# ov2slam/ov2slam

Hardware: AMD Instinct MI355X
Metric: frames/sec tracking + local-BA iters/sec, EuRoC MH_01 stereo 'accurate', 1 GPU vs CPU ref (higher is better)
Workload: dtype u8/int32 fixed point + f32 (LK), f64 (BA)

## Files before the change

ov2slam_amd/csrc/clahe.hip:

```cpp
#include "common.hpp"
#include "xcd_map.hpp"
#include <math.h>
#include <mutex>
#include <type_traits>

#pragma clang fp contract(off)

__device__ __forceinline__ int c_reflect101(int p, int len)
{
    if (len == 1) return 0;
    while (p < 0 || p >= len) p = p < 0 ? -p : 2 * len - 2 - p;
    return p;
}

struct ClaheParams {
    int w, h, stride, tiles_x, tiles_y, tw, th, clip;
    float lut_scale, inv_tw, inv_th;
    long long src_item_stride, dst_item_stride;
    int dst_stride;
    int border;
    int batch, gx_lut;
    int ysplit;
    int nstrips, nlut;
    long long l1_delta;
    int l1_pitch, l1_w, l1_h;
};

__device__ __forceinline__ void clahe_wave_sync()
{
    __builtin_amdgcn_fence(__ATOMIC_RELEASE, "wavefront");
    __builtin_amdgcn_wave_barrier();
    __builtin_amdgcn_fence(__ATOMIC_ACQUIRE, "wavefront");
}

#define CH_WAVE_DW 256
#define CH_CSTRIDE 264
#define CH_NCOPY 4
#define CH_MULTI_DW (CH_NCOPY * CH_CSTRIDE)
typedef uint32_t c_u32x4 __attribute__((ext_vector_type(4)));

template <int CTRL>
__device__ __forceinline__ int c_dpp0(int v) { return __builtin_amdgcn_update_dpp(0, v, CTRL, 0xF, 0xF, true); }

template <bool SRC_ALIGNED, class StoreLut>
__device__ __forceinline__ void clahe_lut_tiles(const ClaheParams &P, const uint8_t *img, uint32_t *hw, int lane, int t, int t_end, int tstride,
                                                StoreLut store_lut, int ncopy = 1)
{
    const int ntiles = t_end;
    const int sub = lane >> 4, l16 = lane & 15;
    uint32_t *hist = hw + ((lane ^ (lane >> 4)) & (ncopy - 1)) * CH_CSTRIDE;
    const bool fast_geom = P.tw <= 61 && P.th <= 64;
    const uint8_t *img_end = img + (long long)(P.h - 1) * P.stride + P.w;
    const bool same_phase = SRC_ALIGNED || (P.stride & 3) == 0;

    auto tile_fast = [&](int t) { const int xb = (t % P.tiles_x) * P.tw; return fast_geom && 2 * xb + P.tw <= 2 * P.w - 1; };
    const uint32_t lane_off = (uint32_t)(sub * P.stride + 4 * l16);
    auto tile_load = [&](int t, uint32_t (&vv)[16], uint32_t &phs) {
        const int ty = t / P.tiles_x, tx = t - ty * P.tiles_x;
        const int x_begin = tx * P.tw;
        if (SRC_ALIGNED && (ty * P.th + 64 <= P.h) && (long long)P.h * P.stride < (1ll << 31)) {
            const uint32_t ph = (uint32_t)(x_begin & 3);
            phs = ph * 0x55555555u;
            const uint8_t *tp = img + (long long)(ty * P.th) * P.stride + (x_begin & ~3);
            uint32_t off = (4 * l16 < P.tw + (int)ph && (x_begin & ~3) + 4 * l16 < P.w) ? lane_off : (uint32_t)(sub * P.stride);
#pragma unroll
            for (int i = 0; i < 16; i++) {
                vv[i] = *(const uint32_t *)(tp + off);
                off += 4u * (uint32_t)P.stride;
            }
            return;
        }
        const int ybase = ty * P.th + sub;
        phs = 0;
#pragma unroll
        for (int i = 0; i < 16; i++) {
            int y = ybase + 4 * i;
            y = y >= P.h ? 2 * P.h - 2 - y : y;
            y = y < 0 ? 0 : y;
            uint32_t v = 0;
            if (SRC_ALIGNED) {
                const uint32_t ph = (uint32_t)(x_begin & 3);
                phs |= ph << (2 * i);
                if (4 * i + sub < P.th && 4 * l16 < P.tw + (int)ph && (x_begin & ~3) + 4 * l16 < P.w) v = *(const uint32_t *)(img + y * P.stride + (x_begin & ~3) + 4 * l16);
            } else {
                const uint8_t *rp = img + (long long)y * P.stride + x_begin;
                const uint32_t ph = (uint32_t)((size_t)rp & 3);
                phs |= ph << (2 * i);
                const uint8_t *ap = rp - ph + 4 * l16;
                if (4 * i + sub < P.th && 4 * l16 < P.tw + (int)ph && x_begin - (int)ph + 4 * l16 < P.w) {
                    if (ap + 4 <= img_end) v = *(const uint32_t *)ap;
                    else for (int k = 0; k < 4; k++) if (ap + k < img_end) v |= (uint32_t)ap[k] << (8 * k);
                }
            }
            vv[i] = v;
        }
    };

    uint32_t cur[16], cur_ph = 0;
    auto histogram = [&](int th) {
        const int ty = th / P.tiles_x, tx = th - ty * P.tiles_x;
        const int x_begin = tx * P.tw;
        if (ncopy == 1) ((c_u32x4 *)hw)[lane] = (c_u32x4)(0u);
        else for (int q = lane; q < CH_MULTI_DW / 4; q += 64) ((c_u32x4 *)hw)[q] = (c_u32x4)(0u);
        clahe_wave_sync();
        if (tile_fast(th)) {
            const int dbl_lo = 2 * P.w - 2 - (x_begin + P.tw);
            auto wgt = [&](int p) { const int c = x_begin + p; return ((unsigned)p < (unsigned)P.tw && c < P.w) ? ((c > dbl_lo && c <= P.w - 2) ? 2u : 1u) : 0u; };
            const int p_same = 4 * l16 - (int)(cur_ph & 3);
            uint32_t w0 = wgt(p_same), w1 = wgt(p_same + 1), w2 = wgt(p_same + 2), w3 = wgt(p_same + 3);
            bool mine = p_same < P.tw;
#pragma unroll
            for (int i = 0; i < 16; i++) {
                if (!same_phase) {
                    const int p0 = 4 * l16 - (int)((cur_ph >> (2 * i)) & 3);
                    w0 = wgt(p0); w1 = wgt(p0 + 1); w2 = wgt(p0 + 2); w3 = wgt(p0 + 3);
                    mine = p0 < P.tw;
                }
                if (mine && 4 * i + sub < P.th) {
                    const uint32_t v = cur[i];
                    atomicAdd(&hist[v & 0xFF], w0);
                    atomicAdd(&hist[(v >> 8) & 0xFF], w1);
                    atomicAdd(&hist[(v >> 16) & 0xFF], w2);
                    atomicAdd(&hist[v >> 24], w3);
                }
            }
        } else {
            for (int ly = sub; ly < P.th; ly += 4) {
                const uint8_t *row = img + (long long)c_reflect101(ty * P.th + ly, P.h) * P.stride;
                for (int lx = l16; lx < P.tw; lx += 16) atomicAdd(&hist[row[c_reflect101(x_begin + lx, P.w)]], 1u);
            }
        }
    };
    if (t < ntiles) {
        if (tile_fast(t)) tile_load(t, cur, cur_ph);
        histogram(t);
        if (t + tstride < ntiles && tile_fast(t + tstride)) tile_load(t + tstride, cur, cur_ph);
    }
#pragma nounroll
    for (; t < ntiles; t += tstride) {
        clahe_wave_sync();
        int hv[4];
        {
            c_u32x4 q = *(const c_u32x4 *)(hw + 4 * lane);
            for (int c = 1; c < ncopy; c++) q += *(const c_u32x4 *)(hw + c * CH_CSTRIDE + 4 * lane);
            hv[0] = (int)q.x; hv[1] = (int)q.y; hv[2] = (int)q.z; hv[3] = (int)q.w;
        }
        clahe_wave_sync();
        const int tn = t + tstride;
        if (tn < ntiles) {
            histogram(tn);
            if (tn + tstride < ntiles && tile_fast(tn + tstride)) tile_load(tn + tstride, cur, cur_ph);
        }
        if (P.clip > 0) {
            int over = 0;
#pragma unroll
            for (int k = 0; k < 4; k++) { over += max(hv[k] - P.clip, 0); hv[k] = min(hv[k], P.clip); }
            over += c_dpp0<0xB1>(over); over += c_dpp0<0x4E>(over); over += c_dpp0<0x124>(over); over += c_dpp0<0x128>(over);
            const int clipped = __builtin_amdgcn_readlane(over, 0) + __builtin_amdgcn_readlane(over, 16) +
                                __builtin_amdgcn_readlane(over, 32) + __builtin_amdgcn_readlane(over, 48);
            const int batch = clipped >> 8, residual = clipped & 255;
            int step = residual ? (int)(256.0f / (float)residual) : 1;
            int q = (int)((float)(4 * lane) / (float)step), r = 4 * lane - q * step;
#pragma unroll
            for (int k = 0; k < 4; k++) {
                hv[k] += batch + ((residual != 0 && r == 0 && q < residual) ? 1 : 0);
                r++;
                if (r == step) { r = 0; q++; }
            }
        }
        hv[1] += hv[0]; hv[2] += hv[1]; hv[3] += hv[2];
        int v = hv[3];
        v += c_dpp0<0x111>(v); v += c_dpp0<0x112>(v); v += c_dpp0<0x114>(v); v += c_dpp0<0x118>(v);
        const int r0 = __builtin_amdgcn_readlane(v, 15), r1 = __builtin_amdgcn_readlane(v, 31), r2 = __builtin_amdgcn_readlane(v, 47);
        const int rowoff = sub == 0 ? 0 : (sub == 1 ? r0 : (sub == 2 ? r0 + r1 : r0 + r1 + r2));
        const int base = v + rowoff - hv[3];
        uint32_t packed = 0;
#pragma unroll
        for (int k = 0; k < 4; k++) {
            int r = __float2int_rn((float)(hv[k] + base) * P.lut_scale);
            r = r < 0 ? 0 : (r > 255 ? 255 : r);
            packed |= (uint32_t)r << (8 * k);
        }
        store_lut(t, packed);
    }
}

template <bool SRC_ALIGNED>
__global__ __launch_bounds__(256, 4) void k_clahe_lut(ClaheParams P, const uint8_t *__restrict__ src, uint8_t *__restrict__ lut)
{
    __shared__ __attribute__((aligned(16))) uint32_t hist_all[4][CH_MULTI_DW];
    const int wave = __builtin_amdgcn_readfirstlane(threadIdx.x >> 6), lane = threadIdx.x & 63;
    const int ntiles = P.tiles_x * P.tiles_y;
    int b, bx;
    ov2_xcd_map(blockIdx.x, P.gx_lut, P.batch, &b, &bx);
    uint8_t *lb = lut + (long long)b * ntiles * 256 + 4 * lane;
    clahe_lut_tiles<SRC_ALIGNED>(P, src + (long long)b * P.src_item_stride, hist_all[wave], lane, bx * 4 + wave, ntiles, 4 * P.gx_lut,
                                 [&](int t, uint32_t packed) { *(uint32_t *)(lb + (long long)t * 256) = packed; }, CH_NCOPY);
}

#define CLAHE_MAX_CELLS 48
#define CA_UNROLL 6
typedef float c_f32x2 __attribute__((ext_vector_type(2)));

__device__ __forceinline__ float c_ub(uint32_t q, int k) { return (float)((q >> (8 * k)) & 0xFFu); }

template <bool SRC_ALIGNED>
__global__ __launch_bounds__(512) void k_clahe_apply(ClaheParams P, const uint8_t *__restrict__ src, const uint8_t *__restrict__ lut,
                                                     uint8_t *__restrict__ dst)
{
    extern __shared__ __align__(16) unsigned char clahe_smem[];
    const int ncx = P.tiles_x + 1;
    uint32_t *lut4 = (uint32_t *)clahe_smem;
    int cy, b;
    ov2_xcd_map(blockIdx.x, (P.tiles_y + 1) * P.ysplit, P.batch, &b, &cy);
    const int part = cy % P.ysplit;
    cy /= P.ysplit;
    const int tid = threadIdx.x, nthr = blockDim.x;
    const int ty1 = max(cy - 1, 0), ty2 = min(cy, P.tiles_y - 1);
    const uint8_t *L = lut + (long long)b * P.tiles_x * P.tiles_y * 256;
    for (int e = tid; e < ncx * 64; e += nthr) {
        const int cx = e >> 6, v4 = (e & 63) * 4;
        const int tx1 = max(cx - 1, 0), tx2 = min(cx, P.tiles_x - 1);
        const uint32_t a = *(const uint32_t *)(L + (ty1 * P.tiles_x + tx1) * 256 + v4), bb = *(const uint32_t *)(L + (ty1 * P.tiles_x + tx2) * 256 + v4);
        const uint32_t c = *(const uint32_t *)(L + (ty2 * P.tiles_x + tx1) * 256 + v4), d = *(const uint32_t *)(L + (ty2 * P.tiles_x + tx2) * 256 + v4);
        const uint32_t ab01 = __builtin_amdgcn_perm(bb, a, 0x05010400u), ab23 = __builtin_amdgcn_perm(bb, a, 0x07030602u);
        const uint32_t cd01 = __builtin_amdgcn_perm(d, c, 0x05010400u), cd23 = __builtin_amdgcn_perm(d, c, 0x07030602u);
        c_u32x4 o;
        o.x = __builtin_amdgcn_perm(cd01, ab01, 0x05040100u); o.y = __builtin_amdgcn_perm(cd01, ab01, 0x07060302u);
        o.z = __builtin_amdgcn_perm(cd23, ab23, 0x05040100u); o.w = __builtin_amdgcn_perm(cd23, ab23, 0x07060302u);
        *(c_u32x4 *)(lut4 + (cx << 8) + v4) = o;
    }
    __syncthreads();
    int y0 = max(0, (int)floorf(((float)cy - 0.5f) * (float)P.th) - 1), y1 = min(P.h, (int)ceilf(((float)cy + 0.5f) * (float)P.th) + 2);
    while (y0 < y1 && (int)floorf((float)y0 * P.inv_th - 0.5f) + 1 != cy) y0++;
    while (y1 > y0 && (int)floorf((float)(y1 - 1) * P.inv_th - 0.5f) + 1 != cy) y1--;
    if (P.ysplit > 1) {
        const int chunk = (y1 - y0 + P.ysplit - 1) / P.ysplit;
        y0 = min(y1, y0 + part * chunk);
        y1 = min(y1, y0 + chunk);
    }
    const uint8_t *simg = src + (long long)b * P.src_item_stride;
    uint8_t *dimg = dst + (long long)b * P.dst_item_stride;
    const bool dst_aligned = ((P.dst_stride | (int)(size_t)dimg) & 3) == 0;
    constexpr bool src_aligned = SRC_ALIGNED;
    const uint8_t *simg_end = simg + (long long)(P.h - 1) * P.stride + P.w;
    const int ndw = (P.w + 3) >> 2;
    for (int dwi = tid; dwi < ndw; dwi += nthr) {
        const int xb = 4 * dwi;
        float xa[4], xa1[4];
        const uint32_t *lutc[4];
#pragma unroll
        for (int k = 0; k < 4; k++) {
            const int x = min(xb + k, P.w - 1);
            const float txf = (float)x * P.inv_tw - 0.5f;
            const int fx = (int)floorf(txf);
            xa[k] = txf - (float)fx; xa1[k] = 1.0f - xa[k];
            lutc[k] = lut4 + ((fx + 1) << 8);
        }
        const c_f32x2 XA01 = {xa[0], xa[1]}, XA23 = {xa[2], xa[3]}, XB01 = {xa1[0], xa1[1]}, XB23 = {xa1[2], xa1[3]};
        const bool full = dst_aligned && xb + 3 < P.w;
        auto load_rows = [&](int yb, uint32_t (&inr)[CA_UNROLL]) {
#pragma unroll
            for (int u = 0; u < CA_UNROLL; u++) {
                const int y = min(yb + u, y1 - 1);
                const uint8_t *sp = simg + (long long)y * P.stride + xb;
                uint32_t in = 0;
                if (src_aligned) in = *(const uint32_t *)sp;
                else {
                    const uint32_t ph = (uint32_t)((size_t)sp & 3);
                    const uint8_t *ap = sp - ph;
                    if (xb + 3 < P.w && ap + 8 <= simg_end) {
                        const uint32_t lo = *(const uint32_t *)ap, hi = *(const uint32_t *)(ap + 4);
                        in = __builtin_amdgcn_alignbyte(hi, lo, ph);
                    } else for (int k = 0; k < 4; k++) if (xb + k < P.w) in |= (uint32_t)sp[k] << (8 * k);
                }
                inr[u] = in;
            }
        };
        uint32_t inr[CA_UNROLL], nxt[CA_UNROLL];
        if (y0 < y1) load_rows(y0, inr);
        for (int yb = y0; yb < y1; yb += CA_UNROLL) {
            load_rows(yb + CA_UNROLL, nxt);
#pragma unroll
            for (int u = 0; u < CA_UNROLL; u++) {
                const int y = yb + u;
                if (y >= y1) break;
                const float tyf = (float)y * P.inv_th - 0.5f;
                const float ya = tyf - (float)(cy - 1), ya1 = 1.0f - ya;
                const c_f32x2 YA = {ya, ya}, YB = {ya1, ya1};
                uint8_t *drow = dimg + y * P.dst_stride;
                const uint32_t in = inr[u];
                const uint32_t q0 = lutc[0][in & 0xFF], q1 = lutc[1][(in >> 8) & 0xFF], q2 = lutc[2][(in >> 16) & 0xFF], q3 = lutc[3][in >> 24];
                const c_f32x2 A11 = {c_ub(q0, 0), c_ub(q1, 0)}, A12 = {c_ub(q0, 1), c_ub(q1, 1)}, A21 = {c_ub(q0, 2), c_ub(q1, 2)}, A22 = {c_ub(q0, 3), c_ub(q1, 3)};
                const c_f32x2 B11 = {c_ub(q2, 0), c_ub(q3, 0)}, B12 = {c_ub(q2, 1), c_ub(q3, 1)}, B21 = {c_ub(q2, 2), c_ub(q3, 2)}, B22 = {c_ub(q2, 3), c_ub(q3, 3)};
                const c_f32x2 r01 = (A11 * XB01 + A12 * XA01) * YB + (A21 * XB01 + A22 * XA01) * YA;
                const c_f32x2 r23 = (B11 * XB23 + B12 * XA23) * YB + (B21 * XB23 + B22 * XA23) * YA;
                uint32_t out = __builtin_amdgcn_cvt_pk_u8_f32(rintf(r01.x), 0, 0u);
                out = __builtin_amdgcn_cvt_pk_u8_f32(rintf(r01.y), 1, out);
                out = __builtin_amdgcn_cvt_pk_u8_f32(rintf(r23.x), 2, out);
                out = __builtin_amdgcn_cvt_pk_u8_f32(rintf(r23.y), 3, out);
                if (full) *(uint32_t *)(drow + xb) = out;
                else for (int k = 0; k < 4; k++) if (xb + k < P.w) drow[xb + k] = (uint8_t)(out >> (8 * k));
            }
#pragma unroll
            for (int u = 0; u < CA_UNROLL; u++) inr[u] = nxt[u];
        }
    }
    if (P.border > 0) {
        __threadfence_block();
        __syncthreads();
        const int win = P.border, pbl = (win + 3) & ~3, wend = (P.w + win + 3) & ~3, rbeg = P.w & ~3;
        const int ndw_lr = pbl / 4 + ((wend - rbeg) >> 2), ndw_row = (pbl + wend) >> 2;
        auto put = [&](int yt, int ysrc, int c0) {
            const uint8_t *srow = dimg + ysrc * P.dst_stride;
            uint32_t v;
            if (c0 >= 0 && c0 + 3 < P.w) v = *(const uint32_t *)(srow + c0);
            else {
                v = 0;
#pragma unroll
                for (int k = 0; k < 4; k++) {
                    int c = c0 + k;
                    c = c < -win ? -win : (c > P.w + win - 1 ? P.w + win - 1 : c);
                    v |= (uint32_t)srow[c_reflect101(c, P.w)] << (8 * k);
                }
            }
            *(uint32_t *)(dimg + yt * P.dst_stride + c0) = v;
        };
        for (int row = tid >> 3; row < y1 - y0; row += nthr >> 3)
            for (int d = tid & 7; d < ndw_lr; d += 8)
                put(y0 + row, y0 + row, d < pbl / 4 ? 4 * d - pbl : rbeg + 4 * (d - pbl / 4));
        for (int k = max(1, y0); k <= min(win, y1 - 1); k++)
            for (int d = tid; d < ndw_row; d += nthr) put(-k, k, 4 * d - pbl);
        for (int k = max(1, P.h - y1); k <= min(win, P.h - 1 - y0); k++)
            for (int d = tid; d < ndw_row; d += nthr) put(P.h - 1 + k, P.h - 1 - k, 4 * d - pbl);
    }
}

__device__ __forceinline__ uint32_t c_wave_shr1(uint32_t v) { return (uint32_t)__builtin_amdgcn_update_dpp(0, (int)v, 0x138, 0xF, 0xF, true); }
__device__ __forceinline__ uint32_t c_wave_shl1(uint32_t v) { return (uint32_t)__builtin_amdgcn_update_dpp(0, (int)v, 0x130, 0xF, 0xF, true); }

#define CS_UNROLL 6
#define CS_MAX_STRIPS 8
#define CS_LUT_PRIO 3
template <bool UNAL, bool FUSED>
__global__ __launch_bounds__(64 * (CS_MAX_STRIPS + 2), 6) void k_clahe_apply_pyr(ClaheParams P, const uint8_t *__restrict__ src, const uint8_t *__restrict__ lut,
                                                                                uint8_t *__restrict__ dst)
{
    extern __shared__ __align__(16) unsigned char clahe_smem[];
    uint32_t *lut4 = (uint32_t *)clahe_smem;
    uint8_t *ring = clahe_smem + (size_t)(P.tiles_x + 1) * 1024;
    const int b = blockIdx.x, s = __builtin_amdgcn_readfirstlane(threadIdx.x >> 6);
    const int lane = threadIdx.x & 63, ndw = (P.w + 3) >> 2, wr = UNAL ? (P.w & 3) : 0;
    uint32_t *hist_w = (uint32_t *)(ring + (size_t)2 * P.tiles_x * 256) + (s < P.nstrips ? s * CH_WAVE_DW : P.nstrips * CH_WAVE_DW + (s - P.nstrips) * CH_MULTI_DW);
    const int hist_copies = s < P.nstrips ? 1 : CH_NCOPY;
    auto lut_row = [&](int ty, int tx0, int txstep) {
        uint8_t *slot = ring + (size_t)(ty & 1) * P.tiles_x * 256 - (size_t)ty * P.tiles_x * 256 + 4 * lane;
        clahe_lut_tiles<!UNAL>(P, src + (long long)b * P.src_item_stride, hist_w, lane, ty * P.tiles_x + tx0, (ty + 1) * P.tiles_x, txstep,
                               [&](int t, uint32_t packed) { *(uint32_t *)(slot + (size_t)t * 256) = packed; }, hist_copies);
    };
    typedef uint32_t cs_u32_a1 __attribute__((aligned(1)));
    const int cmin = 0, ncell = P.tiles_x + 1;
    const uint8_t *L = lut + (long long)b * P.tiles_x * P.tiles_y * 256;
    auto cell_row = [&](int y) { return (int)floorf((float)y * P.inv_th - 0.5f) + 1; };
    int cy = -1, y_switch = 0;
    auto build = [&](int cyv) {
        const int ty1 = max(cyv - 1, 0), ty2 = min(cyv, P.tiles_y - 1);
        const uint8_t *L1 = FUSED ? ring + (size_t)(ty1 & 1) * P.tiles_x * 256 : L + (size_t)ty1 * P.tiles_x * 256;
        const uint8_t *L2 = FUSED ? ring + (size_t)(ty2 & 1) * P.tiles_x * 256 : L + (size_t)ty2 * P.tiles_x * 256;
        __syncthreads();
        for (int e = threadIdx.x; e < ncell * 64; e += blockDim.x) {
            const int cx = cmin + (e >> 6), v4 = (e & 63) * 4;
            const int tx1 = max(cx - 1, 0), tx2 = min(cx, P.tiles_x - 1);
            const uint32_t a = *(const uint32_t *)(L1 + tx1 * 256 + v4), bb = *(const uint32_t *)(L1 + tx2 * 256 + v4);
            const uint32_t c = *(const uint32_t *)(L2 + tx1 * 256 + v4), dd = *(const uint32_t *)(L2 + tx2 * 256 + v4);
            const uint32_t ab01 = __builtin_amdgcn_perm(bb, a, 0x05010400u), ab23 = __builtin_amdgcn_perm(bb, a, 0x07030602u);
            const uint32_t cd01 = __builtin_amdgcn_perm(dd, c, 0x05010400u), cd23 = __builtin_amdgcn_perm(dd, c, 0x07030602u);
            c_u32x4 o;
            o.x = __builtin_amdgcn_perm(cd01, ab01, 0x05040100u); o.y = __builtin_amdgcn_perm(cd01, ab01, 0x07060302u);
            o.z = __builtin_amdgcn_perm(cd23, ab23, 0x05040100u); o.w = __builtin_amdgcn_perm(cd23, ab23, 0x07060302u);
            *(c_u32x4 *)(lut4 + ((e >> 6) << 8) + v4) = o;
        }
        __syncthreads();
    };
    if (FUSED) {
        lut_row(0, s, P.nstrips + P.nlut);
        if (s >= P.nstrips) {
            const int n_cell_rows = cell_row(P.h - 1) + 1;
            __builtin_amdgcn_s_setprio(CS_LUT_PRIO);
            for (int c = 0; c < n_cell_rows; c++) {
                build(c);
                if (c + 1 < P.tiles_y) lut_row(c + 1, s - P.nstrips, P.nlut);
            }
            return;
        }
    }
    const int core0 = s == 0 ? 0 : 63 + 62 * (s - 1);
    const int core1 = s == P.nstrips - 1 ? ndw : 63 + 62 * s;
    const int d_first = s == 0 ? 0 : core0 - 1;
    const int d_raw = d_first + lane;
    const int d = min(d_raw, ndw - 1);
    const bool core = d_raw >= core0 && d_raw < core1;
    const int xb = 4 * d;
    float xa[4], xa1[4];
    const uint32_t *lutc[4];
#pragma unroll
    for (int k = 0; k < 4; k++) {
        const float txf = (float)min(xb + k, P.w - 1) * P.inv_tw - 0.5f;
        const int fx = (int)floorf(txf);
        xa[k] = txf - (float)fx; xa1[k] = 1.0f - xa[k];
        lutc[k] = lut4 + ((fx + 1 - cmin) << 8);
    }
    const c_f32x2 XA01 = {xa[0], xa[1]}, XA23 = {xa[2], xa[3]}, XB01 = {xa1[0], xa1[1]}, XB23 = {xa1[2], xa1[3]};
    uint8_t *dimg = dst + (long long)b * P.dst_item_stride;
    uint8_t *l1 = dimg + P.l1_delta;
    const int win = P.border;
    const int l1odd = UNAL ? (P.l1_w & 1) : 0;
    const int nb0 = (win + 3) >> 2, nb1 = (win + 1) >> 1;
    const int nbr0 = nb0 + (wr ? 1 : 0), nbr1 = nb1 + l1odd;
    const bool bl0 = core && d < nb0, br0 = core && d >= ndw - nbr0;
    const bool bl1 = core && d >= 1 && d <= nb1, br1 = core && d >= ndw - nbr1;
    const bool edge_strip = s == 0 || core1 > ndw - max(nbr0, nbr1);
    const bool first_col = d_raw == 0, last_col = d_raw == ndw - 1;
    const bool dup = d_raw > ndw - 1;
    const uint32_t pad0 = 4u * nb0, pad1 = 2u * nb1;
    const uint32_t slack0 = pad0 + 4u * (uint32_t)((P.w + win + 3) >> 2), slack1 = pad1 + 2u * (uint32_t)((P.l1_w + win + 3) >> 1);
    const uint32_t o0 = dup ? slack0 : pad0 + 4u * d;
    const uint32_t o0b = bl0 ? pad0 - 4u * (d + 1) : (br0 ? pad0 + (uint32_t)(2 * P.w - 2 - xb - ((wr & 1) ? 0 : 2)) : slack0);
    const uint32_t sel_br = (wr & 1) ? 0x01020304u : 0x03040506u;
    const uint32_t sel_fix = (last_col && wr) ? (wr == 1 ? 0x01020304u : (wr == 2 ? 0x03040504u : 0x05060504u)) : 0x07060504u;
    const uint32_t sel_rt = wr == 0 ? 0x0c0c0c06u : (wr == 1 ? 0x0c0c0c00u : (wr == 2 ? 0x0c0c0c02u : 0x0c0c0c04u));
    const uint32_t o1 = core ? pad1 + 2u * d : slack1;
    const uint32_t o1b = bl1 ? pad1 - 2u * d : (br1 ? pad1 + (uint32_t)P.l1_w + 2u * (ndw - 1 - d) - (uint32_t)l1odd : slack1);
    const bool fix1 = last_col && l1odd;
    uint8_t *d0m = dimg - pad0, *d1m = l1 - pad1;
    const uint32_t xo = (d == ndw - 1 && wr) ? (uint32_t)(P.w - 4) : (uint32_t)xb;
    const uint32_t in_sh = (d == ndw - 1 && wr) ? 8u * (4u - (uint32_t)wr) : 0u;

    auto stage = [&](int y) {
        cy = cell_row(y);
        int yn = max(y + 1, (int)(((float)cy + 0.5f) * (float)P.th) - 2);
        while (yn < P.h && cell_row(yn) == cy) yn++;
        y_switch = yn;
        build(cy);
    };
    uint8_t *dbase = min(d0m - (long long)win * P.dst_stride, d1m - (long long)win * P.l1_pitch) - 256;
    const __amdgpu_buffer_rsrc_t rs_dst = __builtin_amdgcn_make_buffer_rsrc(dbase, 0, 0x7fffffff, 0x00020000);
    const uint8_t *sbase = src + (long long)b * P.src_item_stride;
    const __amdgpu_buffer_rsrc_t rs_src = __builtin_amdgcn_make_buffer_rsrc((void *)sbase, 0, 0x7fffffff, 0x00020000);
    auto put0 = [&](uint8_t *row, uint32_t v, uint32_t bv) {
        const int so = (int)(row - dbase);
        __builtin_amdgcn_raw_buffer_store_b32(v, rs_dst, (int)o0, so, 0);
        if (edge_strip) __builtin_amdgcn_raw_buffer_store_b32(bv, rs_dst, (int)o0b, so, 0);
    };
    auto put1 = [&](uint8_t *row, uint32_t v, uint32_t bv) {
        const int so = (int)(row - dbase);
        __builtin_amdgcn_raw_buffer_store_b16((unsigned short)v, rs_dst, (int)o1, so, 0);
        if (edge_strip) __builtin_amdgcn_raw_buffer_store_b16((unsigned short)bv, rs_dst, (int)o1b, so, 0);
    };
    typedef unsigned short cu16x2 __attribute__((ext_vector_type(2)));
    uint8_t *r1 = d1m;
    auto emit = [&](int Y, uint32_t c0, uint32_t c1, uint32_t c2, uint32_t c3, uint32_t c4, auto mirror_c) {
        constexpr bool MIRROR = decltype(mirror_c)::value;
        const cu16x2 s0 = __builtin_bit_cast(cu16x2, c0), s1 = __builtin_bit_cast(cu16x2, c1), s2 = __builtin_bit_cast(cu16x2, c2),
                     s3 = __builtin_bit_cast(cu16x2, c3), s4 = __builtin_bit_cast(cu16x2, c4);
        const cu16x2 v = (s2 * (unsigned short)6 + (s1 + s3) * (unsigned short)4 + s0 + s4 + (unsigned short)128) >> (unsigned short)8;
        uint32_t o = __builtin_amdgcn_perm(0u, __builtin_bit_cast(uint32_t, v), 0x0c0c0200u);
        uint32_t bv = 0;
        if (edge_strip) {
            bv = __builtin_amdgcn_perm(c_wave_shr1(o), o, 0x0c0c0500u);
            if (UNAL && fix1) o = bv;
        }
        put1(r1, o, bv);
        r1 += P.l1_pitch;
        if (MIRROR) {
            if (Y >= 1 && Y <= win) put1(d1m - (long long)Y * P.l1_pitch, o, bv);
            if (Y >= P.l1_h - 1 - win && Y <= P.l1_h - 2) put1(d1m + (long long)(2 * (P.l1_h - 1) - Y) * P.l1_pitch, o, bv);
        }
    };

    uint32_t hA = 0, hB = 0, hC = 0, hD = 0, hE = 0;
    const uint8_t *srow = src + (long long)b * P.src_item_stride;
    uint8_t *r0 = d0m;
    uint32_t inr[CS_UNROLL], nxt[CS_UNROLL];
#pragma unroll
    for (int u = 0; u < CS_UNROLL; u++) inr[u] = *(const cs_u32_a1 *)(srow + (long long)min(u, P.h - 1) * P.stride + xo) >> (UNAL ? in_sh : 0u);
    srow += (long long)CS_UNROLL * P.stride;
    auto do_row = [&](int y, uint32_t in, auto mirror_c) {
        constexpr bool MIRROR = decltype(mirror_c)::value;
        const float tyf = (float)y * P.inv_th - 0.5f;
        const float ya = tyf - (float)(cy - 1), ya1 = 1.0f - ya;
        const c_f32x2 YA = {ya, ya}, YB = {ya1, ya1};
        const uint32_t q0 = lutc[0][in & 0xFF], q1 = lutc[1][(in >> 8) & 0xFF], q2 = lutc[2][(in >> 16) & 0xFF], q3 = lutc[3][in >> 24];
        const c_f32x2 A11 = {c_ub(q0, 0), c_ub(q1, 0)}, A12 = {c_ub(q0, 1), c_ub(q1, 1)}, A21 = {c_ub(q0, 2), c_ub(q1, 2)}, A22 = {c_ub(q0, 3), c_ub(q1, 3)};
        const c_f32x2 B11 = {c_ub(q2, 0), c_ub(q3, 0)}, B12 = {c_ub(q2, 1), c_ub(q3, 1)}, B21 = {c_ub(q2, 2), c_ub(q3, 2)}, B22 = {c_ub(q2, 3), c_ub(q3, 3)};
        const c_f32x2 r01 = (A11 * XB01 + A12 * XA01) * YB + (A21 * XB01 + A22 * XA01) * YA;
        const c_f32x2 r23 = (B11 * XB23 + B12 * XA23) * YB + (B21 * XB23 + B22 * XA23) * YA;
        const c_f32x2 MAGIC = {12582912.0f, 12582912.0f};
        const c_f32x2 m01 = r01 + MAGIC, m23 = r23 + MAGIC;
        const uint32_t u0 = __builtin_bit_cast(uint32_t, (float)m01.x), u1 = __builtin_bit_cast(uint32_t, (float)m01.y);
        const uint32_t u2 = __builtin_bit_cast(uint32_t, (float)m23.x), u3 = __builtin_bit_cast(uint32_t, (float)m23.y);
        uint32_t out = __builtin_amdgcn_perm(__builtin_amdgcn_perm(u3, u2, 0x0c0c0400u), __builtin_amdgcn_perm(u1, u0, 0x0c0c0400u), 0x05040100u);
        uint32_t lf = c_wave_shr1(out), rt = c_wave_shl1(out);
        if (first_col) lf = __builtin_amdgcn_perm(out, out, 0x01020000u);
        if (edge_strip) {
            if (UNAL) out = __builtin_amdgcn_perm(out, lf, sel_fix);
        }
        if (UNAL) { if (last_col) rt = __builtin_amdgcn_perm(out, lf, sel_rt); }
        else if (last_col) rt = out >> 16;
        uint32_t bv = 0;
        if (edge_strip)
            bv = bl0 ? __builtin_amdgcn_perm(out, rt, 0x05060700u) : __builtin_amdgcn_perm(out, lf, sel_br);
        put0(r0, out, bv);
        r0 += P.dst_stride;
        if (MIRROR) {
            if (y >= 1 && y <= win) put0(d0m - (long long)y * P.dst_stride, out, bv);
            if (y >= P.h - 1 - win && y <= P.h - 2) put0(d0m + (long long)(2 * (P.h - 1) - y) * P.dst_stride, out, bv);
        }
        const uint32_t l0 = __builtin_amdgcn_alignbyte(out, lf, 2);
        const uint32_t h0 = __builtin_amdgcn_udot4(l0, 0x04060401u, __builtin_amdgcn_udot4(out, 0x00010000u, 0u, false), false);
        const uint32_t h1 = __builtin_amdgcn_udot4(out, 0x04060401u, __builtin_amdgcn_udot4(rt, 0x00000001u, 0u, false), false);
        hA = hB; hB = hC; hC = hD; hD = hE; hE = h0 | (h1 << 16);
    };
    for (int yb = 0; yb < P.h; yb += CS_UNROLL) {
        if (yb + 2 * CS_UNROLL <= P.h) {
#pragma unroll
            for (int u = 0; u < CS_UNROLL; u++) { nxt[u] = (uint32_t)__builtin_amdgcn_raw_buffer_load_b32(rs_src, (int)xo, (int)(srow - sbase), 0) >> (UNAL ? in_sh : 0u); srow += P.stride; }
        } else {
#pragma unroll
            for (int u = 0; u < CS_UNROLL; u++)
                nxt[u] = *(const cs_u32_a1 *)(src + (long long)b * P.src_item_stride + (long long)min(yb + CS_UNROLL + u, P.h - 1) * P.stride + xo) >> (UNAL ? in_sh : 0u);
        }
        if (yb == y_switch) stage(yb);
        const bool fast = yb > 2 * win + 2 && yb + CS_UNROLL - 1 < P.h - 1 - win && yb + CS_UNROLL - 4 < 2 * (P.l1_h - 1 - win) &&
                          y_switch >= yb + CS_UNROLL && yb + CS_UNROLL <= P.h;
        if (fast) {
#pragma unroll
            for (int u = 0; u < CS_UNROLL; u++) {
                do_row(yb + u, inr[u], std::false_type());
                if ((u & 1) == 0) emit((yb + u - 2) >> 1, hA, hB, hC, hD, hE, std::false_type());
            }
        } else {
#pragma nounroll
            for (int u = 0; u < CS_UNROLL; u++) {
                const int y = yb + u;
                if (y >= P.h) break;
                if (y == y_switch) stage(y);
                do_row(y, inr[0], std::true_type());
                if (!(y & 1)) {
                    if (y == 2) emit(0, hE, hD, hC, hD, hE, std::true_type());
                    else if (y > 2) emit((y - 2) >> 1, hA, hB, hC, hD, hE, std::true_type());
                }
#pragma unroll
                for (int k = 0; k + 1 < CS_UNROLL; k++) inr[k] = inr[k + 1];
            }
        }
#pragma unroll
        for (int u = 0; u < CS_UNROLL; u++) inr[u] = nxt[u];
    }
    if (P.h & 1) emit((P.h - 1) >> 1, hC, hD, hE, hD, hC, std::true_type());
    else emit((P.h - 2) >> 1, hB, hC, hD, hE, hD, std::true_type());
}

int ov2_launch_clahe(ov2_ctx *ctx, const uint8_t *src_d, int w, int h, int stride, size_t src_batch_stride, int batch,
                     double clip_limit, int tiles_x, int tiles_y, uint8_t *dst_d, int dst_stride, size_t dst_batch_stride,
                     uint8_t *lut_d, int border, const PyrDesc *pyr, int *level1_done)
{
    if (level1_done) *level1_done = 0;
    OV2_REQUIRE(tiles_x + 1 <= CLAHE_MAX_CELLS && (size_t)(tiles_x + 1) * 1024 <= 160 * 1024, OV2_EUNSUPPORTED,
                "CLAHE: too many tile columns / too wide an image for the LDS tables");
    static std::once_flag attr_once;
    static hipError_t attr_err = hipSuccess;
    std::call_once(attr_once, [] {
        attr_err = hipFuncSetAttribute((const void *)k_clahe_apply<true>, hipFuncAttributeMaxDynamicSharedMemorySize, 160 * 1024);
        if (attr_err == hipSuccess)
            attr_err = hipFuncSetAttribute((const void *)k_clahe_apply<false>, hipFuncAttributeMaxDynamicSharedMemorySize, 160 * 1024);
    });
    OV2_HIP_CHECK(attr_err);
    ClaheParams P;
    P.border = border;
    P.nstrips = 0; P.nlut = 0; P.l1_delta = 0; P.l1_pitch = P.l1_w = P.l1_h = 0;
    int ew = w, eh = h;
    if (!(w % tiles_x == 0 && h % tiles_y == 0)) { ew = w + (tiles_x - w % tiles_x); eh = h + (tiles_y - h % tiles_y); }
    P.w = w; P.h = h; P.stride = stride; P.tiles_x = tiles_x; P.tiles_y = tiles_y;
    P.tw = ew / tiles_x; P.th = eh / tiles_y;
    const int total = P.tw * P.th;
    P.lut_scale = (float)(256 - 1) / (float)total;
    P.clip = 0;
    if (clip_limit > 0.0) { P.clip = (int)(clip_limit * total / 256); if (P.clip < 1) P.clip = 1; }
    P.inv_tw = 1.0f / (float)P.tw; P.inv_th = 1.0f / (float)P.th;
    P.src_item_stride = (long long)src_batch_stride; P.dst_item_stride = (long long)dst_batch_stride; P.dst_stride = dst_stride;
    const int tiles_per_wave = (long long)batch * tiles_x * tiles_y >= 32768 ? 5 : 1;
    const bool src_al = ((stride | (int)(size_t)src_d | (int)src_batch_stride) & 3) == 0;
    P.ysplit = (long long)batch * (tiles_y + 1) >= 256 ? 1 : (P.th >= 48 ? 6 : (P.th >= 16 ? 3 : 1));
    P.batch = batch; P.gx_lut = (tiles_x * tiles_y + 4 * tiles_per_wave - 1) / (4 * tiles_per_wave);
    bool lut_launched = false;
    auto launch_lut = [&] {
        if (!lut_launched) hipLaunchKernelGGL(src_al ? k_clahe_lut<true> : k_clahe_lut<false>, dim3(P.gx_lut * batch), dim3(256), 0, ctx->stream, P, src_d, lut_d);
        lut_launched = true;
    };
    if (pyr && pyr->n_levels >= 2 && border == pyr->win && w >= 64 && h >= 8 && 2 * ((border + 3) / 4) + 1 <= (w + 3) / 4 &&
        (((size_t)dst_d | (size_t)dst_stride | dst_batch_stride) & 3) == 0 && (pyr->lv[1].img_pitch & 1) == 0) {
        const int ndw = (w + 3) / 4, nstrips = ndw <= 64 ? 1 : 2 + (ndw - 126 + 61) / 62;
        const bool want = ctx->clahe_strips >= 0 ? ctx->clahe_strips >= 1 : (long long)batch * nstrips >= 1024;
        if (want && nstrips <= CS_MAX_STRIPS && tiles_x + 1 <= 40) {
            static std::once_flag strip_once;
            static hipError_t strip_err = hipSuccess;
            std::call_once(strip_once, [] {
                const void *fn[4] = {(const void *)k_clahe_apply_pyr<false, false>, (const void *)k_clahe_apply_pyr<true, false>,
                                     (const void *)k_clahe_apply_pyr<false, true>, (const void *)k_clahe_apply_pyr<true, true>};
                for (int i = 0; i < 4 && strip_err == hipSuccess; i++) strip_err = hipFuncSetAttribute(fn[i], hipFuncAttributeMaxDynamicSharedMemorySize, 72 * 1024);
            });
            OV2_HIP_CHECK(strip_err);
            P.nstrips = nstrips;
            P.l1_delta = pyr->lv[1].img_roi - pyr->lv[0].img_roi; P.l1_pitch = pyr->lv[1].img_pitch; P.l1_w = pyr->lv[1].w; P.l1_h = pyr->lv[1].h;
            const bool unal = (w & 3) != 0 || (pyr->lv[1].w & 1) != 0;
            const int nlut = tiles_x <= 16 ? 1 : std::max(1, std::min((tiles_x + 7) / 8, CS_MAX_STRIPS + 2 - nstrips));
            const bool fused = (ctx->clahe_strips == 2 || (ctx->clahe_strips < 0 && tiles_x <= 16 * nlut)) && (unal || src_al);
            if (fused) {
                P.nlut = nlut;
                const size_t lds = (size_t)(tiles_x + 1) * 1024 + (size_t)2 * tiles_x * 256 + ((size_t)nstrips * CH_WAVE_DW + (size_t)P.nlut * CH_MULTI_DW) * 4;
                hipLaunchKernelGGL((unal ? k_clahe_apply_pyr<true, true> : k_clahe_apply_pyr<false, true>), dim3(batch), dim3(64 * (nstrips + P.nlut)), lds, ctx->stream, P, src_d, lut_d, dst_d);
            } else {
                launch_lut();
                hipLaunchKernelGGL((unal ? k_clahe_apply_pyr<true, false> : k_clahe_apply_pyr<false, false>), dim3(batch), dim3(64 * nstrips), (size_t)(tiles_x + 1) * 1024, ctx->stream, P, src_d, lut_d, dst_d);
            }
            OV2_HIP_CHECK(hipGetLastError());
            if (level1_done) *level1_done = 1;
            return OV2_OK;
        }
    }
    launch_lut();
    const size_t apply_lds = (size_t)(tiles_x + 1) * 1024;
    const int ndw = (w + 3) / 4, passes = (ndw + 511) / 512;
    const int apply_threads = (((ndw + passes - 1) / passes) + 63) / 64 * 64;
    hipLaunchKernelGGL(src_al ? k_clahe_apply<true> : k_clahe_apply<false>, dim3((tiles_y + 1) * P.ysplit * batch), dim3(apply_threads), apply_lds, ctx->stream, P, src_d, lut_d, dst_d);
    OV2_HIP_CHECK(hipGetLastError());
    return OV2_OK;
}

extern "C" {

int ov2_clahe_d(ov2_ctx *ctx, const uint8_t *src_d, int w, int h, int stride, size_t src_batch_stride, int batch,
                double clip_limit, int tiles_x, int tiles_y, uint8_t *dst_d, int dst_stride, size_t dst_batch_stride)
{
    OV2_REQUIRE(ctx && src_d && dst_d, OV2_EINVAL, "NULL argument");
    OV2_REQUIRE(w > 0 && h > 0 && stride >= w && dst_stride >= w && batch >= 1 && tiles_x > 0 && tiles_y > 0, OV2_EINVAL, "bad geometry");
    OV2_REQUIRE(tiles_x <= w && tiles_y <= h, OV2_EINVAL, "more tiles than pixels");
    OV2_HIP_CHECK(hipSetDevice(ctx->device));
    const size_t lut_bytes = (size_t)batch * tiles_x * tiles_y * 256;
    const int rc = ctx->reserve_device(lut_bytes);
    if (rc != OV2_OK) return rc;
    return ov2_launch_clahe(ctx, src_d, w, h, stride, src_batch_stride, batch, clip_limit, tiles_x, tiles_y, dst_d, dst_stride,
                            dst_batch_stride, (uint8_t *)ctx->d_scratch, 0, nullptr, nullptr);
}

int ov2_pyr_build_clahe_d(ov2_ctx *ctx, ov2_pyr *p, const uint8_t *img_d, int stride, size_t img_batch_stride,
                          double clip_limit, int tiles_x, int tiles_y)
{
    OV2_REQUIRE(ctx && p && img_d, OV2_EINVAL, "NULL argument");
    OV2_REQUIRE(stride >= p->w && tiles_x > 0 && tiles_y > 0 && tiles_x <= p->w && tiles_y <= p->h, OV2_EINVAL, "bad geometry");
    OV2_REQUIRE(p->d.batch == 1 || img_batch_stride >= (size_t)stride * (size_t)p->h, OV2_EINVAL, "img_batch_stride too small");
    OV2_HIP_CHECK(hipSetDevice(ctx->device));
    const size_t lut_bytes = (size_t)p->d.batch * tiles_x * tiles_y * 256;
    int rc = ctx->reserve_device(lut_bytes);
    if (rc != OV2_OK) return rc;
    const PyrLevelDesc &L0 = p->d.lv[0];
    int l1_done = 0;
    rc = ov2_launch_clahe(ctx, img_d, p->w, p->h, stride, img_batch_stride, p->d.batch, clip_limit, tiles_x, tiles_y,
                          p->d.base + L0.img_roi, L0.img_pitch, (size_t)p->d.item_stride, (uint8_t *)ctx->d_scratch, p->d.win,
                          &p->d, &l1_done);
    if (rc != OV2_OK) return rc;
    rc = ov2_launch_pyr_build(ctx, p, nullptr, 0, 0, l1_done);
    if (rc != OV2_OK) return rc;
    return ov2_pyr_mark_ready(ctx, p);
}

int ov2_pyr_build_clahe_h(ov2_ctx *ctx, ov2_pyr *p, const uint8_t *img_h, int stride, double clip_limit, int tiles_x, int tiles_y)
{
    OV2_REQUIRE(ctx && p && img_h, OV2_EINVAL, "NULL argument");
    OV2_REQUIRE(p->d.batch == 1, OV2_EINVAL, "host-buffer entry point takes batch=1 pyramids");
    OV2_REQUIRE(stride >= p->w && tiles_x > 0 && tiles_y > 0 && tiles_x <= p->w && tiles_y <= p->h, OV2_EINVAL, "bad geometry");
    OV2_HIP_CHECK(hipSetDevice(ctx->device));
    const size_t pitch = ((size_t)p->w + 15) & ~(size_t)15;
    const size_t img = (pitch * p->h + 255) & ~(size_t)255, lut_bytes = (size_t)tiles_x * tiles_y * 256;
    int rc = ctx->reserve_device(img + lut_bytes);
    if (rc != OV2_OK) return rc;
    uint8_t *ds = (uint8_t *)ctx->d_scratch;
    rc = ctx->upload_image(ds, pitch, img_h, (size_t)stride, (size_t)p->w, (size_t)p->h);
    if (rc != OV2_OK) return rc;
    const PyrLevelDesc &L0 = p->d.lv[0];
    int l1_done = 0;
    rc = ov2_launch_clahe(ctx, ds, p->w, p->h, (int)pitch, 0, 1, clip_limit, tiles_x, tiles_y, p->d.base + L0.img_roi, L0.img_pitch,
                          (size_t)p->d.item_stride, ds + img, p->d.win, &p->d, &l1_done);
    if (rc != OV2_OK) return rc;
    rc = ov2_launch_pyr_build(ctx, p, nullptr, 0, 0, l1_done);
    if (rc != OV2_OK) return rc;
    return ov2_pyr_mark_ready(ctx, p);
}

int ov2_pyr_build_clahe_hb(ov2_ctx *ctx, ov2_pyr *p, int n_items, const uint8_t *const *img_h, int stride, double clip_limit, int tiles_x, int tiles_y)
{
    OV2_REQUIRE(ctx && p && img_h, OV2_EINVAL, "NULL argument");
    OV2_REQUIRE(p->parent == nullptr, OV2_EINVAL, "an item view is read-only");
    OV2_REQUIRE(n_items >= 1 && n_items <= p->d.batch, OV2_EINVAL, "n_items out of range");
    const bool use_clahe = clip_limit >= 0.0;
    OV2_REQUIRE(stride >= p->w && (!use_clahe || (tiles_x > 0 && tiles_y > 0 && tiles_x <= p->w && tiles_y <= p->h)), OV2_EINVAL, "bad geometry");
    for (int b = 0; b < n_items; b++) OV2_REQUIRE(img_h[b] != nullptr, OV2_EINVAL, "NULL image");
    OV2_HIP_CHECK(hipSetDevice(ctx->device));
    const size_t pitch = ((size_t)p->w + 15) & ~(size_t)15;
    const size_t img = (pitch * p->h + 255) & ~(size_t)255, lut_bytes = use_clahe ? (size_t)n_items * tiles_x * tiles_y * 256 : 0;
    int rc = ctx->reserve_device(img * (size_t)n_items + lut_bytes);
    if (rc != OV2_OK) return rc;
    uint8_t *ds = (uint8_t *)ctx->d_scratch;
    rc = ctx->upload_images(ds, pitch, img, img_h, n_items, (size_t)stride, (size_t)p->w, (size_t)p->h);
    if (rc != OV2_OK) return rc;
    ov2_pyr q = *p;
    q.d.batch = n_items;
    if (use_clahe) {
        const PyrLevelDesc &L0 = q.d.lv[0];
        int l1_done = 0;
        rc = ov2_launch_clahe(ctx, ds, p->w, p->h, (int)pitch, img, n_items, clip_limit, tiles_x, tiles_y, q.d.base + L0.img_roi, L0.img_pitch,
                              (size_t)q.d.item_stride, ds + img * (size_t)n_items, q.d.win, &q.d, &l1_done);
        if (rc != OV2_OK) return rc;
        rc = ov2_launch_pyr_build(ctx, &q, nullptr, 0, 0, l1_done);
    } else
        rc = ov2_launch_pyr_build(ctx, &q, ds, (int)pitch, img);
    if (rc != OV2_OK) return rc;
    return ov2_pyr_mark_ready(ctx, p);
}

int ov2_clahe_h(ov2_ctx *ctx, const uint8_t *src_h, int w, int h, int stride, double clip_limit, int tiles_x, int tiles_y,
                uint8_t *dst_h, int dst_stride)
{
    OV2_REQUIRE(ctx && src_h && dst_h, OV2_EINVAL, "NULL argument");
    OV2_REQUIRE(w > 0 && h > 0 && stride >= w && dst_stride >= w && tiles_x > 0 && tiles_y > 0, OV2_EINVAL, "bad geometry");
    OV2_REQUIRE(tiles_x <= w && tiles_y <= h, OV2_EINVAL, "more tiles than pixels");
    OV2_HIP_CHECK(hipSetDevice(ctx->device));
    const size_t pitch = ((size_t)w + 15) & ~(size_t)15;
    const size_t img = (pitch * h + 255) & ~(size_t)255, lut_bytes = (size_t)tiles_x * tiles_y * 256;
    int rc = ctx->reserve_device(2 * img + lut_bytes);
    if (rc != OV2_OK) return rc;
    uint8_t *ds = (uint8_t *)ctx->d_scratch;
    rc = ctx->upload_image(ds, pitch, src_h, (size_t)stride, (size_t)w, (size_t)h);
    if (rc != OV2_OK) return rc;
    const int rc2 = ov2_launch_clahe(ctx, ds, w, h, (int)pitch, 0, 1, clip_limit, tiles_x, tiles_y, ds + img, (int)pitch, 0, ds + 2 * img, 0, nullptr, nullptr);
    if (rc2 != OV2_OK) return rc2;
    rc = ctx->download_image(dst_h, (size_t)dst_stride, ds + img, pitch, (size_t)w, (size_t)h);
    if (rc != OV2_OK) return rc;
    return OV2_OK;
}

}
```

Before: 1.056 million.

## Shrink fused CLAHE LDS footprint by single-buffering LUT ring and aliasing histograms

Reorganises the fused CLAHE kernel's shared memory. The two-row LUT ring becomes a single row, and the bilinear cell table is built incrementally: the previous row's values are reused from the existing entries instead of being re-read from a second ring slot. Strip histograms are aliased onto the cell-table region when they fit. This cuts LDS per block so more blocks can be resident per CU. It also adds incremental-update and aliasing hazards, since correctness now depends on the build order and on the synchronisation between the histogram and cell-table phases.

```diff
diff --git a/ov2slam_amd/csrc/clahe.hip b/ov2slam_amd/csrc/clahe.hip
--- a/ov2slam_amd/csrc/clahe.hip
+++ b/ov2slam_amd/csrc/clahe.hip
@@ -1,5 +1,6 @@
 #include "common.hpp"
 #include "xcd_map.hpp"
+#include "clahe_lds.hpp"
 #include <math.h>
 #include <mutex>
 #include <type_traits>
@@ -33,10 +34,6 @@
     __builtin_amdgcn_fence(__ATOMIC_ACQUIRE, "wavefront");
 }
 
-#define CH_WAVE_DW 256
-#define CH_CSTRIDE 264
-#define CH_NCOPY 4
-#define CH_MULTI_DW (CH_NCOPY * CH_CSTRIDE)
 typedef uint32_t c_u32x4 __attribute__((ext_vector_type(4)));
 
 template <int CTRL>
@@ -347,14 +344,15 @@
                                                                                 uint8_t *__restrict__ dst)
 {
     extern __shared__ __align__(16) unsigned char clahe_smem[];
-    uint32_t *lut4 = (uint32_t *)clahe_smem;
-    uint8_t *ring = clahe_smem + (size_t)(P.tiles_x + 1) * 1024;
+    const ClaheFusedLds lds = clahe_fused_lds(P.tiles_x, P.nstrips, P.nlut);
+    uint32_t *lut4 = (uint32_t *)(clahe_smem + lds.lut4);
+    uint8_t *ring = clahe_smem + lds.ring;
     const int b = blockIdx.x, s = __builtin_amdgcn_readfirstlane(threadIdx.x >> 6);
     const int lane = threadIdx.x & 63, ndw = (P.w + 3) >> 2, wr = UNAL ? (P.w & 3) : 0;
-    uint32_t *hist_w = (uint32_t *)(ring + (size_t)2 * P.tiles_x * 256) + (s < P.nstrips ? s * CH_WAVE_DW : P.nstrips * CH_WAVE_DW + (s - P.nstrips) * CH_MULTI_DW);
+    uint32_t *hist_w = s < P.nstrips ? (uint32_t *)(clahe_smem + lds.hist_strip) + s * CH_WAVE_DW : (uint32_t *)(clahe_smem + lds.hist_lut) + (s - P.nstrips) * CH_MULTI_DW;
     const int hist_copies = s < P.nstrips ? 1 : CH_NCOPY;
     auto lut_row = [&](int ty, int tx0, int txstep) {
-        uint8_t *slot = ring + (size_t)(ty & 1) * P.tiles_x * 256 - (size_t)ty * P.tiles_x * 256 + 4 * lane;
+        uint8_t *slot = ring - (size_t)ty * P.tiles_x * 256 + 4 * lane;
         clahe_lut_tiles<!UNAL>(P, src + (long long)b * P.src_item_stride, hist_w, lane, ty * P.tiles_x + tx0, (ty + 1) * P.tiles_x, txstep,
                                [&](int t, uint32_t packed) { *(uint32_t *)(slot + (size_t)t * 256) = packed; }, hist_copies);
     };
@@ -365,12 +363,33 @@
     int cy = -1, y_switch = 0;
     auto build = [&](int cyv) {
         const int ty1 = max(cyv - 1, 0), ty2 = min(cyv, P.tiles_y - 1);
-        const uint8_t *L1 = FUSED ? ring + (size_t)(ty1 & 1) * P.tiles_x * 256 : L + (size_t)ty1 * P.tiles_x * 256;
-        const uint8_t *L2 = FUSED ? ring + (size_t)(ty2 & 1) * P.tiles_x * 256 : L + (size_t)ty2 * P.tiles_x * 256;
+        const uint8_t *L1 = L + (size_t)ty1 * P.tiles_x * 256, *L2 = L + (size_t)ty2 * P.tiles_x * 256;
         __syncthreads();
         for (int e = threadIdx.x; e < ncell * 64; e += blockDim.x) {
             const int cx = cmin + (e >> 6), v4 = (e & 63) * 4;
             const int tx1 = max(cx - 1, 0), tx2 = min(cx, P.tiles_x - 1);
+            if (FUSED) {
+                c_u32x4 *ent = (c_u32x4 *)(lut4 + ((e >> 6) << 8) + v4);
+                c_u32x4 o;
+                if (cyv >= P.tiles_y) {
+                    const c_u32x4 q = *ent;
+                    o.x = __builtin_amdgcn_perm(q.x, q.x, 0x03020302u); o.y = __builtin_amdgcn_perm(q.y, q.y, 0x03020302u);
+                    o.z = __builtin_amdgcn_perm(q.z, q.z, 0x03020302u); o.w = __builtin_amdgcn_perm(q.w, q.w, 0x03020302u);
+                } else {
+                    const uint32_t c = *(const uint32_t *)(ring + tx1 * 256 + v4), dd = *(const uint32_t *)(ring + tx2 * 256 + v4);
+                    const uint32_t cd01 = __builtin_amdgcn_perm(dd, c, 0x05010400u), cd23 = __builtin_amdgcn_perm(dd, c, 0x07030602u);
+                    if (cyv == 0) {
+                        o.x = __builtin_amdgcn_perm(cd01, cd01, 0x05040100u); o.y = __builtin_amdgcn_perm(cd01, cd01, 0x07060302u);
+                        o.z = __builtin_amdgcn_perm(cd23, cd23, 0x05040100u); o.w = __builtin_amdgcn_perm(cd23, cd23, 0x07060302u);
+                    } else {
+                        const c_u32x4 q = *ent;
+                        o.x = __builtin_amdgcn_perm(cd01, q.x, 0x05040302u); o.y = __builtin_amdgcn_perm(cd01, q.y, 0x07060302u);
+                        o.z = __builtin_amdgcn_perm(cd23, q.z, 0x05040302u); o.w = __builtin_amdgcn_perm(cd23, q.w, 0x07060302u);
+                    }
+                }
+                *ent = o;
+                continue;
+            }
             const uint32_t a = *(const uint32_t *)(L1 + tx1 * 256 + v4), bb = *(const uint32_t *)(L1 + tx2 * 256 + v4);
             const uint32_t c = *(const uint32_t *)(L2 + tx1 * 256 + v4), dd = *(const uint32_t *)(L2 + tx2 * 256 + v4);
             const uint32_t ab01 = __builtin_amdgcn_perm(bb, a, 0x05010400u), ab23 = __builtin_amdgcn_perm(bb, a, 0x07030602u);
@@ -618,7 +637,7 @@
             const bool fused = (ctx->clahe_strips == 2 || (ctx->clahe_strips < 0 && tiles_x <= 16 * nlut)) && (unal || src_al);
             if (fused) {
                 P.nlut = nlut;
-                const size_t lds = (size_t)(tiles_x + 1) * 1024 + (size_t)2 * tiles_x * 256 + ((size_t)nstrips * CH_WAVE_DW + (size_t)P.nlut * CH_MULTI_DW) * 4;
+                const size_t lds = clahe_fused_lds(tiles_x, nstrips, P.nlut).bytes;
                 hipLaunchKernelGGL((unal ? k_clahe_apply_pyr<true, true> : k_clahe_apply_pyr<false, true>), dim3(batch), dim3(64 * (nstrips + P.nlut)), lds, ctx->stream, P, src_d, lut_d, dst_d);
             } else {
                 launch_lut();
diff --git a/ov2slam_amd/csrc/clahe_lds.hpp b/ov2slam_amd/csrc/clahe_lds.hpp
--- /dev/null
+++ b/ov2slam_amd/csrc/clahe_lds.hpp
@@ -0,0 +1,32 @@
+#pragma once
+#include <stddef.h>
+
+#define CH_WAVE_DW 256
+#define CH_CSTRIDE 264
+#define CH_NCOPY 4
+#define CH_MULTI_DW (CH_NCOPY * CH_CSTRIDE)
+
+#define CS_LDS_PER_CU 163840
+#define CS_LDS_GRANULE 128
+
+struct ClaheFusedLds {
+    size_t lut4, ring, hist_strip, hist_lut, bytes;
+};
+
+constexpr ClaheFusedLds clahe_fused_lds(int tiles_x, int nstrips, int nlut)
+{
+    ClaheFusedLds l{};
+    l.lut4 = 0;
+    l.ring = l.lut4 + (size_t)(tiles_x + 1) * 1024;
+    const size_t after_ring = l.ring + (size_t)tiles_x * 256;
+    const bool inside = nstrips <= tiles_x + 1;
+    l.hist_strip = inside ? l.lut4 : after_ring;
+    l.hist_lut = inside ? after_ring : after_ring + (size_t)nstrips * CH_WAVE_DW * 4;
+    l.bytes = l.hist_lut + (size_t)nlut * CH_MULTI_DW * 4;
+    return l;
+}
+
+constexpr int clahe_fused_lds_residents(int tiles_x, int nstrips, int nlut)
+{
+    return (int)(CS_LDS_PER_CU / ((clahe_fused_lds(tiles_x, nstrips, nlut).bytes + CS_LDS_GRANULE - 1) / CS_LDS_GRANULE * CS_LDS_GRANULE));
+}
```

Result: no change. 1.060 million (median of 6 runs) (+0.4%).
